# uniio/ivf-hnsw

Measured on AMD Instinct MI355X. Metric: queries/sec @ Recall@1, SIFT1B PQ16 nprobe=32; ADC scan HBM GB/s vs peak, higher is better.
Workload: dtype f32

## Files before the change

### ivf-hnsw_amd/csrc/capi_internal.h

```cpp
#pragma once
#include "../../include/ivfhnsw_hip.h"
#include "ivfhnsw_kernels.h"

#include <hip/hip_runtime.h>

#include <algorithm>
#include <new>
#include <cmath>
#include <cstddef>
#include <cstdio>
#include <cstdlib>
#include <cstring>
#include <functional>
#include <string>
#include <unordered_map>
#include <vector>

namespace ivfhnsw_gpu_impl {

int fail(int code, const char *fmt, ...) __attribute__((format(printf, 2, 3)));

#define HIP_TRY(expr)                                                                                        \
    do {                                                                                                     \
        hipError_t e_ = (expr);                                                                              \
// ... 98 lines not shown
};

struct StatusWords {
    uint32_t bits;
    uint32_t walk_next;
    uint32_t redo_len;
    uint32_t redo_next;
    uint32_t redo_exits;
    uint32_t heap_redo_len;
    uint32_t heap_redo_exits;
    uint32_t pad;
};
static_assert(offsetof(StatusWords, redo_len) == offsetof(StatusWords, walk_next) + 4 &&
                  offsetof(StatusWords, redo_next) == offsetof(StatusWords, walk_next) + 8 &&
                  offsetof(StatusWords, redo_exits) == offsetof(StatusWords, walk_next) + 12,
              "launch_coarse: next_query is followed by the three words of the redo header");
static_assert(offsetof(StatusWords, heap_redo_exits) == offsetof(StatusWords, heap_redo_len) + 4, "launch_heap_scan: redo_hdr[0..1]");
static_assert(offsetof(StatusWords, bits) == 0 && sizeof(StatusWords) == 8 * sizeof(uint32_t), "8 words, bits first");

struct WalkScratch {
    bool zero = false;
    void *zero_ptr = nullptr;
    size_t zero_bytes = 0;
    bool counters_clean = true;
};

}

using namespace ivfhnsw_gpu_impl;

#define IVFHNSW_GPU_DEVBUFS(X) \
    X(goff) X(loff) X(cnorm) X(pqc) X(ntab) X(opq_at) X(opq_a) X(codes) X(ncodes) X(ids)  \
    X(g_alpha) X(g_nn) X(g_sizes) X(g_inter)  \
    X(q_counts) X(q_links) X(q_vectors) X(q_qrows) X(q_nbrows) X(q_nbnorms) X(q_fat) X(q_links_c)  \
    X(e_pqc) X(e_ntab) X(e_a) X(e_at) X(e_x) X(e_idx) X(e_dist) X(e_res) X(e_tmp) X(e_codes) X(e_ncodes)  \
    X(t_x) X(t_y) X(t_cb) X(t_assign) X(t_part) X(t_c)  \
    X(k_q) X(k_x) X(k_qn) X(k_xn) X(k_part) X(k_ids) X(k_dists)  \
    X(km_x) X(km_c) X(km_assign) X(km_dist) X(km_cnt) X(km_start) X(km_ids) X(km_ids2) X(km_hist) X(km_part) X(km_status) X(km_pairs)  \
    X(gb_table) X(gb_fwd) X(gb_fcnt) X(gb_deg) X(gb_roff) X(gb_ids) X(gb_ids2) X(gb_hist) X(gb_stat) X(gb_counts) X(gb_links)  \
    X(cg_q) X(cg_cidx) X(cg_ids) X(cg_dists) X(gc_nn) X(cg_cvn) X(cg_tab) X(cg_tab2) X(cg_off) X(cg_alpha2) X(cg_sub)  \
    X(base_rows) X(base_stage)  \
    X(r_q) X(r_cand) X(r_dist) X(r_lab)  \
    X(ex_q) X(ex_part) X(ex_raw) X(ex_dist) X(ex_lab)  \
    X(ap_idx) X(ap_ids) X(ap_codes) X(ap_ncodes) X(ap_cnt) X(ap_own) X(ap_part) X(ap_status) X(ap_perm) X(ap_perm2) X(ap_hist) X(ap_tiles)  \
    X(gp_sub) X(gp_sizes) X(gp_pre_old) X(gp_pre_new) X(gp_rows) X(gp_gather) X(ga_cidx) X(ga_off) X(ga_nn) X(ga_alpha) X(ga_inter) X(ga_status)  \
    X(rm_labels) X(rm_bits) X(rm_mask) X(rm_keep) X(rm_rem) X(rm_out) X(rm_part) X(rm_status) X(rm_sizes)  \
    X(f_mask) X(f_count)  \
    X(fs_planes) X(fs_count) X(fs_qslots)  \
    X(tg_table) X(tg_rows)  \
    X(bf_words) X(bf_rows) X(bf_own) X(bf_count)  \
    X(bs_table) X(bs_plan) X(bs_qslots)  \
    X(bt_tags) X(bt_rows) X(bt_off) X(bt_work)  \
    X(w_xq) X(w_luts) X(w_segs) X(w_lpos) X(w_hdr) X(w_keys) X(w_cid) X(w_cd) X(w_qsd) X(w_totals) X(w_visited) X(w_status) X(w_stream) X(w_slen) X(w_tail) X(w_redo) X(w_hredo) X(w_heap)  \
    X(rg_dist) X(rg_lab) X(rg_slices) X(rg_part) X(rg_lims)  \
    X(xr_dist) X(xr_lab) X(xr_slices) X(xr_part) X(xr_map) X(xr_lims) X(xr_tot)  \
    X(lc_bits) X(lc_labels) X(lc_sorted) X(lc_perm) X(lc_perm2) X(lc_hist) X(lc_lo) X(lc_cnt) X(lc_rows) X(lc_counts) X(lc_scalar)  \
    X(rc_rows) X(rc_y) X(rc_out) X(sr_keys) X(sr_rows)  \
    X(s_q) X(s_cid) X(s_cd) X(s_dist) X(s_lab) X(s_keys) X(s_len)

struct ivfhnsw_gpu {
    int device = 0;
    hipStream_t stream = nullptr;
    bool own_stream = false;
    bool is_view = false;

#define IVFHNSW_X(name) DevBuf name;
    IVFHNSW_GPU_DEVBUFS(IVFHNSW_X)
// ... 320 lines not shown
```

### ivf-hnsw_amd/csrc/capi_upload.cpp

```cpp
#include "capi_internal.h"
#include "walk_form.h"

namespace {

int check_desc(const ivfhnsw_ivf_desc *d, bool need_lists)
{
    if (!d)
        return fail(IVFHNSW_ERR_INVALID, "null descriptor");
    if (d->d == 0 || d->nc == 0 || d->code_size == 0)
        return fail(IVFHNSW_ERR_INVALID, "d, nc and code_size must be positive");
    if (d->code_size % 4)
        return fail(IVFHNSW_ERR_INVALID, "code_size %zu is not a multiple of 4 (IndexIVF_HNSW.cpp:805)", d->code_size);
    if (d->code_size * 1024 > kScanDynLdsMax)
        return fail(IVFHNSW_ERR_INVALID, "code_size %zu: the query's table (1 KB per code byte) must fit %zu KB of LDS",
                    d->code_size, kScanDynLdsMax / 1024);
    if (d->d % d->code_size)
        return fail(IVFHNSW_ERR_INVALID, "d %zu is not a multiple of code_size %zu", d->d, d->code_size);
    if (d->d / d->code_size > 64)
        return fail(IVFHNSW_ERR_INVALID, "sub-vector dimension %zu > 64 unsupported", d->d / d->code_size);
    if (d->nc >= 0xffffffffull)
        return fail(IVFHNSW_ERR_INVALID, "nc too large");
    if (!d->offsets || !d->centroid_norms || !d->pq_centroids || !d->norm_table)
        return fail(IVFHNSW_ERR_INVALID, "offsets, centroid_norms, pq_centroids and norm_table are required");
    if (need_lists && d->offsets[d->nc] != 0 && (!d->ids || !d->codes || !d->norm_codes))
        return fail(IVFHNSW_ERR_INVALID, "ids, codes and norm_codes are required");
    if (d->shard_world == 0 || d->shard_rank >= d->shard_world)
        return fail(IVFHNSW_ERR_INVALID, "bad shard %u of %u", d->shard_rank, d->shard_world);
    if (d->offsets[0] != 0)
        return fail(IVFHNSW_ERR_INVALID, "offsets[0] must be 0");
    for (size_t c = 0; c < d->nc; c++)
        if (d->offsets[c + 1] < d->offsets[c])
            return fail(IVFHNSW_ERR_INVALID, "offsets not monotone at list %zu", c);
    return IVFHNSW_OK;
// ... 251 lines not shown
    h->g.nsubc = (int)nsubc;
    h->g.alphas = h->g_alpha.as<float>();
    h->g.nn_idx = h->g_nn.as<uint32_t>();
    h->g.sub_sizes = h->g_sizes.as<uint32_t>();
    h->g.inter_dists = h->g_inter.as<float>();
    h->g.dedupe = grouping_dedupe(nc, nsubc, subgroup_sizes, nn_centroid_idxs);
    h->has_group = true;
    return IVFHNSW_OK;
} catch (const std::bad_alloc &) {
    return fail(IVFHNSW_ERR_NOMEM, "ivfhnsw_gpu_upload_grouping: host allocation failed");
}

static int build_byte_rows(ivfhnsw_gpu *h, size_t n, size_t d, const float *vectors)
{
    static const bool off = [] {
        const char *e = getenv("IVFHNSW_WALK_PREFILTER");
        return e && atoi(e) == 0;
    }();
    if (off || d > 2048)
        return IVFHNSW_OK;
    float lo = vectors[0], hi = vectors[0];
    bool finite = true;
    for (size_t i = 0; i < n * d; i++) {
        const float v = vectors[i];
        finite &= std::isfinite(v);
        lo = std::min(lo, v);
        hi = std::max(hi, v);
    }
    const float step = (float)(((double)hi - (double)lo) / 255.0);
    if (!finite || !(step > 0.f) || !std::isfinite(step) || !std::isfinite(1.f / step))
        return IVFHNSW_OK;
    std::vector<uint8_t> rows(n * d);
    double worst = 0.0;
    for (size_t r = 0; r < n; r++) {
        double e2 = 0.0;
        for (size_t j = 0; j < d; j++) {
            const double x = vectors[r * d + j];
            double c = std::nearbyint((x - (double)lo) / (double)step);
            c = std::min(255.0, std::max(0.0, c));
            rows[r * d + j] = (uint8_t)c;
            const double e = x - ((double)lo + (double)step * c);
            e2 += e * e;
        }
        worst = std::max(worst, e2);
    }
    const double errc = std::sqrt(worst) / (double)step * (1.0 + 1e-6) + 1e-6;
    float errc_f = (float)errc;
    if ((double)errc_f < errc)
        errc_f = std::nextafter(errc_f, INFINITY);
    int rc = upload(h->q_qrows, rows.data(), n * d);
    if (rc)
        return rc;
    h->gr.qrows = h->q_qrows.as<uint8_t>();
    h->gr.q_lo = lo;
    h->gr.q_step = step;
    h->gr.q_errc = errc_f;
    return IVFHNSW_OK;
}

static int build_neighbour_rows(ivfhnsw_gpu *h)
{
    static const int mode = [] {
        const char *e = getenv("IVFHNSW_WALK_PREFILTER");
        return e ? atoi(e) : 2;
    }();
    static const double cap_gib = [] {
        const char *e = getenv("IVFHNSW_WALK_NBROWS_GIB");
        return e ? atof(e) : 48.0;
    }();
    if (!h->gr.qrows || mode != 2 || h->gr.d > 128 || h->gr.n >= (1u << 24) || h->gr.maxM > 64)
        return IVFHNSW_OK;
    const int nb_rows = (h->gr.maxM + 31) & ~31;
    const size_t bytes = (size_t)h->gr.n * nb_rows * 128;
    if ((double)bytes > cap_gib * 1073741824.0)
        return IVFHNSW_OK;
    int rc = h->q_nbrows.ensure(bytes);
    if (rc)
        return rc;
    if ((rc = h->q_nbnorms.ensure((size_t)h->gr.n * nb_rows * sizeof(uint32_t))))
        return rc;
    if ((rc = h->q_links_c.ensure((size_t)h->gr.n * h->gr.maxM * sizeof(uint32_t))))
        return rc;
    HIP_TRY(launch_build_nbrows(h->stream, h->gr, h->q_nbrows.as<uint8_t>(), h->q_nbnorms.as<uint32_t>(), nb_rows,
                                h->q_links_c.as<uint32_t>()));
    HIP_TRY(hipStreamSynchronize(h->stream));
    h->gr.nbrows = h->q_nbrows.as<uint8_t>();
    h->gr.nbnorms = h->q_nbnorms.as<uint32_t>();
    h->gr.links_c = h->q_links_c.as<uint32_t>();
    h->gr.nb_rows = nb_rows;
    return IVFHNSW_OK;
}

int ivfhnsw_gpu_upload_quantizer(ivfhnsw_gpu *h, size_t n, size_t d, size_t maxM, uint32_t enterpoint,
                                 const uint8_t *link_counts, const uint32_t *links, const float *vectors)
try {
    int rc = table_change_guard(h, kUploads, "upload_quantizer", false);
    if (rc)
        return rc;
    if (n == 0 || d == 0 || maxM == 0 || maxM > 255 || n >= 0xffffffffull || enterpoint >= n || !link_counts ||
        !links || !vectors)
        return fail(IVFHNSW_ERR_INVALID, "bad quantizer arrays (n %zu, d %zu, maxM %zu)", n, d, maxM);
    if (d % 16)
        return fail(IVFHNSW_ERR_INVALID, "d %zu: the reference distance ignores dims beyond a multiple of 16 "
                                         "(hnswalg.cpp:330); only multiples of 16 are supported here", d);
    bool unique = true;
    uint32_t tmp[256];
    for (size_t i = 0; i < n; i++) {
        if (link_counts[i] > maxM)
            return fail(IVFHNSW_ERR_INVALID, "node %zu has %u links > maxM %zu", i, link_counts[i], maxM);
        for (size_t j = 0; j < link_counts[i]; j++)
            if (links[i * maxM + j] >= n)
                return fail(IVFHNSW_ERR_INVALID, "node %zu link %zu out of range", i, j);
        if (unique && link_counts[i] > 1) {
            const size_t c = link_counts[i];
            std::copy(links + i * maxM, links + i * maxM + c, tmp);
            std::sort(tmp, tmp + c);
            unique = std::adjacent_find(tmp, tmp + c) == tmp + c;
// ... 29 lines not shown
    if ((rc = upload(h->q_vectors, vectors, n * d * sizeof(float))))
        return rc;
    h->gr.n = (uint32_t)n;
    h->gr.d = (int)d;
    h->gr.maxM = (int)maxM;
    h->gr.enterpoint = enterpoint;
    h->gr.counts = h->q_counts.as<uint8_t>();
    h->gr.links = h->q_links.as<uint32_t>();
    h->gr.vectors = h->q_vectors.as<float>();
    {
        static const int merge = [] {
            const char *e = getenv("IVFHNSW_WALK_MERGE");
            return (e && atoi(e) == 0) ? 0 : 1;
        }();
        h->gr.merge_admissions = merge;
    }
    {
        static const int late_knob = [] {
            const char *e = getenv("IVFHNSW_WALK_LATE_VISIT");
            return e ? (atoi(e) != 0 ? 1 : 0) : -1;
        }();
        const bool late = late_knob < 0 ? walk_late_visit_default(n) : late_knob == 1;
        h->gr.links_unique = (unique && late) ? 1 : 0;
    }
    h->gr.fat = nullptr;
    h->gr.qrows = nullptr;
    h->gr.nbrows = nullptr;
    h->gr.nbnorms = nullptr;
    h->gr.links_c = nullptr;
    h->gr.nb_rows = 0;
    h->gr.q_lo = 0.f;
    h->gr.q_step = 1.f;
    h->gr.q_errc = 0.f;
    if ((rc = build_byte_rows(h, n, d, vectors)))
        return rc;
    if ((rc = build_neighbour_rows(h)))
        return rc;
    h->has_graph = true;
    return IVFHNSW_OK;
} catch (const std::bad_alloc &) {
    return fail(IVFHNSW_ERR_NOMEM, "ivfhnsw_gpu_upload_quantizer: host allocation failed");
}

int ivfhnsw_gpu_prepare_latency(ivfhnsw_gpu *h)
{
    if (h && h->is_view)
        return fail(IVFHNSW_ERR_STATE, "prepare_latency goes to the handle that holds the tables, not to a view of it");
    int rc = bind(h);
    if (rc)
        return rc;
    if (!h->has_graph)
        return fail(IVFHNSW_ERR_STATE, "prepare_latency needs upload_quantizer");
    if (h->gr.fat)
        return IVFHNSW_OK;
    GraphTables probe = h->gr;
    probe.fat = reinterpret_cast<const float *>(h);
    if (!coarse_latency_supported(probe, 1))
        return fail(IVFHNSW_ERR_INVALID, "the latency walk needs d = 128 or 96, maxM <= 32 and at most 2^20 nodes "
                                         "(have d %d, maxM %d, %u nodes); small batches keep the throughput walk",
                    h->gr.d, h->gr.maxM, h->gr.n);
    if ((rc = h->q_fat.ensure(coarse_latency_fat_bytes(h->gr))))
        return rc;
    HIP_TRY(launch_build_fat(h->stream, h->gr, h->q_fat.as<float>()));
    HIP_TRY(hipStreamSynchronize(h->stream));
    h->gr.fat = h->q_fat.as<float>();
    return IVFHNSW_OK;
// ... 68 lines not shown
```

### ivf-hnsw_amd/csrc/ivfhnsw_kernels.h

```cpp
#pragma once

#include <hip/hip_runtime.h>
#include <mutex>
#include <stdint.h>

#include "scan_dispatch.h"
#include "sweep_plan_math.h"
#include "update_math.h"
#include "walk_form.h"

namespace ivfhnsw_gpu_impl {

struct DynLdsState {
    std::mutex m;
    size_t raised[64] = {};
};
inline hipError_t raise_dyn_lds(const void *kern, size_t bytes, DynLdsState &st)
{
    int dev = 0;
    hipError_t e = hipGetDevice(&dev);
    if (e != hipSuccess)
        return e;
    if (dev < 0 || dev >= 64)
        return hipFuncSetAttribute(kern, hipFuncAttributeMaxDynamicSharedMemorySize, (int)bytes);
// ... 60 lines not shown
struct IvfTables {
    int d, M, dsub;
    uint32_t nc;
    const uint64_t *goff;
    const uint32_t *loff;
    const float *centroid_norms;
    const float *pq_centroids;
    const float *norm_table;
    const float *opq_At;
    const uint8_t *codes;
    const uint8_t *norm_codes;
    const uint32_t *ids;
    uint32_t shard_rank, shard_world;
};

struct GroupTables {
    int nsubc;
    const float *alphas;
    const uint32_t *nn_idx;
    const uint32_t *sub_sizes;
    const float *inter_dists;
    int dedupe;
};

struct GraphTables {
    uint32_t n;
    int d, maxM;
    uint32_t enterpoint;
    const uint8_t *counts;
    const uint32_t *links;
    const float *vectors;
    const uint8_t *qrows;
    float q_lo, q_step, q_errc;
    const uint8_t *nbrows;
    const uint32_t *nbnorms;
    const uint32_t *links_c;
    int nb_rows;
    const float *fat;
    int visited_clean;
    int merge_admissions;
    int links_unique;
};

hipError_t launch_opq(hipStream_t s, const float *At, const float *x, float *y, int nq, int d);
hipError_t launch_lut(hipStream_t s, const IvfTables &t, const float *xq, float *luts, int nq, const PlanHdr *hdr = nullptr);
hipError_t launch_plan_ivf(hipStream_t s, const IvfTables &t, const uint32_t *coarse_ids, const float *coarse_dists,
                           int nprobe, uint64_t max_codes, const PlanView &p, uint64_t *keys, int k);
hipError_t launch_plan_lut(hipStream_t s, const IvfTables &t, const float *xq, const uint32_t *coarse_ids,
                           const float *coarse_dists, int nprobe, uint64_t max_codes, const PlanView &p, uint64_t *keys,
                           int k, float *luts);
hipError_t launch_plan_grouping(hipStream_t s, const IvfTables &t, const GroupTables &g, const GraphTables &gr,
                                const float *xq, const uint32_t *coarse_ids, const float *coarse_dists, int nprobe,
                                uint64_t max_codes, int do_pruning, const PlanView &p, uint64_t *keys, int k,
                                float *qsd_scratch);
struct ScanOut {
    uint64_t *stream = nullptr;
    uint32_t *stream_len = nullptr;
    uint32_t stream_cap = 0;
    float *sel_dist = nullptr;
    int64_t *sel_labels = nullptr;
};
hipError_t launch_scan(hipStream_t s, const IvfTables &t, const float *luts, const PlanView &p, int k, int nsplit,
                       uint64_t *keys, int seg_len_hint, const ScanFilter &fmask, const ScanOut &out, bool *did_select,
                       const char **kernel_name);
bool scan_pipe_supported(const IvfTables &t, int max_seg, int nq, int nsplit, bool has_codes, bool forced = false);
hipError_t launch_scan_pipe(hipStream_t s, const IvfTables &t, const float *xq, const PlanView &p, uint64_t *keys);
// ... 55 lines not shown
                               uint32_t *cnt, double *part, uint32_t *status);
hipError_t launch_scan_u32(hipStream_t s, const uint32_t *in, uint32_t *out, size_t len);
hipError_t launch_sort_by_key(hipStream_t s, const uint32_t *keys, size_t n, int key_bits, uint32_t *ids_a, uint32_t *ids_b,
                              uint32_t *hist, uint32_t **sorted);
hipError_t launch_sort_by_key_from(hipStream_t s, const uint32_t *keys, size_t n, int key_bits, const uint32_t *start,
                                   uint32_t *ids_a, uint32_t *ids_b, uint32_t *hist, uint32_t **sorted);
hipError_t launch_kmeans_means(hipStream_t s, const float *x, size_t n, const uint32_t *members, const uint32_t *start,
                               const uint32_t *cnt, float *c, size_t nc, int d);
hipError_t launch_kmeans_split(hipStream_t s, float *c, const uint32_t *pairs, size_t npairs, int d);
inline int knn_splits_for(size_t nq, size_t nx) { return sweep_splits_for(nq, nx, 128); }
hipError_t launch_knn_norms(hipStream_t s, const float *x, float *out, size_t n, int d);
hipError_t launch_knn(hipStream_t s, const float *Q, const float *X, const float *qn, const float *xn, size_t nq, size_t nx,
                      int d, int k, int mode, int nsplit, unsigned long long *part, uint32_t *ids, float *dists);
size_t graph_forward_lds_bytes(int d, int ncand);
size_t graph_fold_lds_bytes(int d, int maxM);
hipError_t launch_graph_forward(hipStream_t s, const float *x, const uint32_t *table, size_t n, int d, int M, int ncand,
                                uint32_t *fwd, uint8_t *fcnt, uint32_t *deg);
hipError_t launch_graph_fold(hipStream_t s, const float *x, const uint32_t *fwd, const uint8_t *fcnt, const uint32_t *roff,
                             const uint32_t *pairs, size_t n, int d, int M, int maxM, uint8_t *counts, uint32_t *links,
                             uint32_t *longest);
hipError_t launch_group_table(hipStream_t s, int mode, const float *vectors, const uint32_t *centroid_idx,
                              const uint32_t *nn, const float *alphas, const float *cv_in, float *out, size_t ngroups,
                              int nsubc, int d);
size_t group_points_lds_bytes(int nsubc, int d);
hipError_t launch_group_points(hipStream_t s, int mode, const float *vectors, const uint32_t *centroid_idx,
                               const float *table, const float *cv_norms, const unsigned long long *offsets,
                               const float *x, float *out_num, float *out_den, uint32_t *out_sub, size_t ngroups,
                               int nsubc, int d);
hipError_t launch_group_alpha(hipStream_t s, const unsigned long long *offsets, const float *num, const float *den,
                              float *alphas, size_t ngroups);
hipError_t launch_group_rows(hipStream_t s, const unsigned long long *offsets, const uint32_t *sub, uint32_t *rows,
                             size_t ngroups, int nsubc);
hipError_t launch_build_nbrows(hipStream_t s, const GraphTables &g, uint8_t *nbrows, uint32_t *nbnorms, int nb_rows,
                               uint32_t *links_c);
hipError_t launch_fill_bytes(hipStream_t s, uint8_t *dst, size_t nbytes, uint64_t seed);
hipError_t launch_fill_iota(hipStream_t s, uint32_t *dst, size_t n, uint32_t first);
hipError_t launch_fill_lists(hipStream_t s, const IvfTables &t, uint8_t *codes, uint8_t *norm_codes, uint32_t *ids,
                             uint64_t seed_codes, uint64_t seed_norms);
hipError_t launch_rerank_permute(hipStream_t s, const uint8_t *src, size_t src_stride, uint8_t *dst, size_t count, int d);
size_t rerank_lds_bytes(int kc, int d);
hipError_t launch_rerank(hipStream_t s, const uint8_t *base, uint64_t n, int d, const float *queries,
                         const int64_t *cand, size_t nq, int kc, int k, float *dist, int64_t *labels);
inline int exact_rows_per_block(int k) { return k <= 32 ? 128 : 64; }
inline int exact_splits_for(size_t nq, size_t nx, int k) { return sweep_splits_for(nq, nx, exact_rows_per_block(k)); }
hipError_t launch_exact_search(hipStream_t s, const uint8_t *Qp, const uint8_t *X, size_t nq, size_t nx, int d, int k,
                               int nsplit, unsigned long long *part, float *dists, int64_t *labels, const SweepCols &cols = {});
constexpr int kExactRangeMaxShift = 20;
inline int exact_range_map_words(size_t nx, int nsplit, int map_shift) { return sweep_map_words(nx, nsplit, map_shift); }
hipError_t launch_exact_range(hipStream_t s, bool fill, const uint8_t *Qp, const uint8_t *X, size_t nq, size_t q_off, size_t nx,
                              int d, int thr, int nsplit, uint32_t *slices, unsigned long long *total, uint32_t *map,
                              int map_shift, float *dist, int64_t *labels, size_t out_cap, const SweepCols &cols = {});
hipError_t launch_pass_words(hipStream_t s, const uint32_t *bits, size_t bit_words, uint64_t n, int deny, uint32_t *words,
                             unsigned long long *count);
hipError_t launch_pass_rows(hipStream_t s, const uint32_t *words, uint64_t n, uint32_t *cnt, uint32_t *part, uint32_t *rows);
hipError_t launch_strip_plan(hipStream_t s, const uint8_t *d_slots, size_t m, const StripCols *table, void *plan, size_t bound,
                             StripPlan *sp);
hipError_t launch_rerank_permute_rows(hipStream_t s, const uint8_t *src, size_t src_stride, uint8_t *dst, size_t count, int d,
                                      const int32_t *row_src);
hipError_t launch_exact_search_strips(hipStream_t s, const uint8_t *Qp, const uint8_t *X, size_t nq, size_t bound, int d, int k,
                                      int nsplit, unsigned long long *part, float *dists, int64_t *labels, const StripPlan &sp,
                                      unsigned forms);
hipError_t launch_exact_range_strips(hipStream_t s, bool fill, const uint8_t *Qp, const uint8_t *X, size_t bound, size_t q_off,
                                     size_t nx, int d, int thr, int nsplit, uint32_t *slices, unsigned long long *total,
                                     uint32_t *map, int map_shift, float *dist, int64_t *labels, size_t out_cap,
                                     const StripPlan &sp, unsigned forms);
hipError_t launch_base_tags_apply(hipStream_t s, const uint32_t *rows, const uint16_t *vals, size_t cnt, uint64_t n, uint16_t *tags,
                                  uint32_t *conflict);
// ... 74 lines not shown
```

### ivf-hnsw_amd/csrc/kernels_hnsw.hip

```cpp
#include "ivfhnsw_kernels.h"
#include "device_common.h"
#include "walk_set.h"
#include "walk_form.h"

#include <float.h>
#include <stdio.h>
#include <stdlib.h>
#include <type_traits>

namespace ivfhnsw_gpu_impl {


template <int TAGW> struct VisFields {
    static constexpr int cntw = TAGW == 8 ? 8 : TAGW == 10 ? 14 : 16;
    static constexpr int cshift = 64 - cntw;
    static constexpr int slots = cshift / TAGW;
    static constexpr unsigned long long ones()
    {
        unsigned long long o = 0;
        for (int i = 0; i < slots; i++)
            o |= 1ull << (TAGW * i);
        return o;
    }
};

template <int TAGW, int NB>
__device__ __forceinline__ bool visit_test_and_set(uint32_t id, unsigned long long *vt, uint32_t *bm, bool &used_bitmap)
{
    if constexpr (TAGW != 0) {
        using F = VisFields<TAGW>;
        constexpr unsigned long long kOnes = F::ones();
        constexpr unsigned long long kHighs = kOnes << (TAGW - 1);
        const uint32_t b = id % (uint32_t)NB;
        const unsigned long long tag = (unsigned long long)((id / (uint32_t)NB) + 1);
        const unsigned long long old = vt[b];
        const unsigned long long x = old ^ (tag * kOnes);
// ... 66 lines not shown
        __builtin_amdgcn_sched_barrier(0);
#pragma unroll
        for (int i = 0; i < 4; i++) {
            if (j0 + 2 * i < nchunk) {
                const float4 *qq = reinterpret_cast<const float4 *>(sqp + 16 * (j0 + 2 * i));
                const uint32_t ws[4] = {w[i].x, w[i].y, w[i].z, w[i].w};
#pragma unroll
                for (int c = 0; c < 4; c++) {
                    const float4 qv = qq[c];
                    const float t0 = qv.x - (float)(ws[c] & 0xffu);
                    const float t1 = qv.y - (float)((ws[c] >> 8) & 0xffu);
                    const float t2 = qv.z - (float)((ws[c] >> 16) & 0xffu);
                    const float t3 = qv.w - (float)(ws[c] >> 24);
                    a0 = fmaf(t0, t0, a0);
                    a1 = fmaf(t1, t1, a1);
                    a2 = fmaf(t2, t2, a2);
                    a3 = fmaf(t3, t3, a3);
                }
            }
        }
    }
    return (a0 + a1) + (a2 + a3);
}

__device__ __forceinline__ unsigned long long walk_stamp()
{
    __builtin_amdgcn_sched_barrier(0);
    const unsigned long long t = __builtin_amdgcn_s_memtime();
    __builtin_amdgcn_s_waitcnt(0xC07F);
    __builtin_amdgcn_sched_barrier(0);
    return t;
}


struct WalkArgs {
    GraphTables g;
    const float *xq;
    int nq, nprobe, ef;
    uint32_t *coarse_ids;
    float *coarse_dists;
    uint32_t *visited;
    size_t vwords;
    uint32_t *status, *next_query, *redo_hdr, *redo_list;
    uint32_t *tail_bitmaps;
    unsigned long long *stamp_out;
};

template <class T> __device__ __forceinline__ const __attribute__((address_space(4))) T *late_kernarg()
{
    auto p = (const __attribute__((address_space(4))) T *)__builtin_amdgcn_kernarg_segment_ptr();
    asm volatile("" : "+s"(p));
    return p;
}

template <int NCH, int TAGW, int FMODE, bool STAMPS = false, bool SPILL = false, int D = 0, int MAXM = 0, bool MERGE = true>
__global__ __launch_bounds__(64, 4) void hnsw_walk_kernel(WalkArgs a)
{
    constexpr bool SHAPED = D != 0 && MAXM != 0;
    const GraphTables &g = a.g;
    const int ef = a.ef;
    uint32_t *__restrict__ const visited = a.visited;
    const size_t vwords = a.vwords;
#define WALK_COLD(f) (SHAPED ? late_kernarg<WalkArgs>()->f : a.f)
    extern __shared__ __attribute__((aligned(16))) unsigned char smem[];
    float *s_q = reinterpret_cast<float *>(smem);
    static_assert(!SHAPED || (FMODE >= 2 && !SPILL && D % 16 == 0 && D <= 128 && MAXM <= 64),
                  "shape constants go with the neighbour-row forms");
    static_assert(SHAPED || MERGE, "the generic form reads merge_admissions at run time");
    const int dim = D ? D : g.d;
    const int maxm = MAXM ? MAXM : g.maxM;
    const int nbr_rows = MAXM ? (MAXM + 31) / 32 * 32 : g.nb_rows;
    float *s_qp = s_q + dim;
    const int dp = FMODE == 1 ? dim : 0;
    uint32_t *s_q8 = reinterpret_cast<uint32_t *>(s_qp + dp);
    unsigned long long *tail = reinterpret_cast<unsigned long long *>(smem + (size_t)(dim + dp) * sizeof(float) + 512);
    constexpr int NB = walk_vis_buckets(TAGW);
    unsigned long long st_acc[9] = {0, 0, 0, 0, 0, 0}, st_t = 0;
    const int merge_extra = (NCH <= 4 && ef + 8 > kTailCap) ? ef + 8 - kTailCap : 0;
    unsigned long long *vt = tail + kTailCap + merge_extra;
    constexpr bool LDSVIS = TAGW != 0;

    const int lane = threadIdx.x;
    const int judged_row = 8 * (((lane >> 2) & 1) * 2 + (lane & 1)) + (lane >> 3);
    const bool merge_on = SHAPED ? MERGE : g.merge_admissions != 0;
    constexpr bool prefilter = FMODE != 0;
    constexpr bool inline_rows = FMODE >= 2;
    constexpr bool ROWNORMS = FMODE == 3;
    constexpr bool CK = FMODE >= 2;
    auto enc_id = [](uint32_t id, uint32_t c) { return CK ? (id << 7) | c : id; };
    auto dec_id = [](uint32_t e) { return CK ? e >> 7 : e; };
    uint32_t *bm = visited + (size_t)blockIdx.x * vwords;
    TailSpill spill;
    spill.bm = SPILL ? a.tail_bitmaps + (size_t)blockIdx.x * vwords : nullptr;
    spill.hi = -1;
    spill.count = 0;
    bool bitmap_dirty = !(LDSVIS && g.visited_clean);
    bool redo_ran = false;

    for (;;) {
        int q = 0;
        if constexpr (SPILL) {
            if (lane == 0) {
                const uint32_t i = atomicAdd(&a.redo_hdr[1], 1u);
                q = i < a.redo_hdr[0] ? (int)a.redo_list[i] : a.nq;
            }
        } else {
            if (lane == 0)
                q = (int)atomicAdd(WALK_COLD(next_query), 1u);
        }
        q = __builtin_amdgcn_readfirstlane(q);
        if (q >= WALK_COLD(nq))
            break;
        redo_ran = true;
        if (STAMPS)
            st_t = walk_stamp();

        if (!LDSVIS || bitmap_dirty) {
            uint4 *bm4 = reinterpret_cast<uint4 *>(bm);
            const size_t v4 = vwords / 4;
            for (size_t w = lane; w < v4; w += 64)
                bm4[w] = make_uint4(0u, 0u, 0u, 0u);
            bitmap_dirty = false;
        }
        if (LDSVIS)
            for (int w = lane; w < NB; w += 64)
                vt[w] = 0ull;
        __syncthreads();
        float qp_sq = 0.f;
        for (int i = lane; i < dim; i += 64) {
            const float v = WALK_COLD(xq)[(size_t)q * dim + i];
            s_q[i] = v;
            if (prefilter) {
                const float vp = __fdiv_rn(__fsub_rn(v, WALK_COLD(g.q_lo)), g.q_step);
                if (!inline_rows)
                    s_qp[i] = vp;
                qp_sq = fmaf(vp, vp, qp_sq);
            }
        }
        __syncthreads();
        float q_reg[16];
#pragma unroll
        for (int i = 0; i < 16; i++)
            if constexpr (D != 0)
                q_reg[i] = 8 * i < D ? s_q[8 * i + (lane & 7)] : 0.f;
            else
                q_reg[i] = (g.d == 128 || g.d == 96) && 8 * i < g.d ? s_q[8 * i + (lane & 7)] : 0.f;
        float pf_slack = 0.f, pf_slack_q = 0.f, pf_bonus = 0.f;
        int q16_w = 0;
        int x_const = 0;
        bool x_any = false;
        bool x_hi = false;
        uint4 qp_h = make_uint4(0u, 0u, 0u, 0u), qp_l = qp_h, qp_x = qp_h;
        if (prefilter) {
#pragma unroll
            for (int off = 32; off > 0; off >>= 1)
                qp_sq += __shfl_xor(qp_sq, off, 64);
            pf_slack = __uint_as_float(__builtin_amdgcn_readfirstlane(__float_as_uint(WALK_COLD(g.q_errc) + 3.9e-6f * sqrtf(qp_sq))));
            if (inline_rows) {
                float dq_sq = 0.f, bonus = 0.f;
                int s_hh = 0, s_hl = 0, s_ll = 0, s_xh = 0, s_xl = 0;
                if (lane < 32) {
                    uint32_t wh = 0, wl = 0, wxl = 0, wxh = 0;
#pragma unroll
                    for (int b = 0; b < 4; b++) {
                        const int comp = 4 * lane + b;
                        const float vp = comp < dim ? __fdiv_rn(__fsub_rn(s_q[comp], WALK_COLD(g.q_lo)), g.q_step) : 0.f;
                        const float fh = fminf(255.f, fmaxf(0.f, floorf(vp)));
                        const float fl = fminf(255.f, fmaxf(0.f, rintf((vp - fh) * 256.f)));
                        const float qin = fh + fl * 0.00390625f;
                        const bool below = vp < 0.f, above = vp >= 256.f;
                        const float e = (below || above) ? 0.f : vp - qin;
                        dq_sq = fmaf(e, e, dq_sq);
                        const float out = (below || above) ? fabsf(vp - qin) : 0.f;
                        bonus = fmaf(out, out, bonus);
                        const int x = (int)fminf(255.f, floorf(2.f * out));
                        const int hi = (int)fh, lo = (int)fl;
                        s_hh += hi * hi;
                        s_hl += hi * lo;
                        s_ll += lo * lo;
                        wh |= (uint32_t)hi << (8 * b);
                        wl |= (uint32_t)lo << (8 * b);
                        if (below)
                            wxl |= (uint32_t)x << (8 * b);
                        if (above)
                            wxh |= (uint32_t)x << (8 * b);
                        s_xl += below ? x : 0;
                        s_xh += above ? x : 0;
                    }
                    s_q8[lane] = wh;
                    s_q8[32 + lane] = wl;
// ... 202 lines not shown
                        const uint32_t ws[4] = {nw[i].x, nw[i].y, nw[i].z, nw[i].w};
                        uint32_t hr = 0, rr = 0;
#pragma unroll
                        for (int c = 0; c < 4; c++) {
                            hr = __builtin_amdgcn_udot4(qh[c], ws[c], hr, false);
                            if constexpr (!ROWNORMS)
                                rr = __builtin_amdgcn_udot4(ws[c], ws[c], rr, false);
                        }
                        uint32_t lr = hr << 8;
#pragma unroll
                        for (int c = 0; c < 4; c++)
                            lr = __builtin_amdgcn_udot4(ql[c], ws[c], lr, false);
                        S[i] = (int)(128u * rr - lr);
                        X[i] = 0;
                        if (x_any) {
                            uint32_t xlr = 0, xhr = 0;
#pragma unroll
                            for (int c = 0; c < 4; c++)
                                xlr = __builtin_amdgcn_udot4(xl[c], ws[c], xlr, false);
                            if (x_hi) {
                                asm volatile("" ::);
#pragma unroll
                                for (int c = 0; c < 4; c++)
                                    xhr = __builtin_amdgcn_udot4(xh[c], ws[c], xhr, false);
                            }
                            X[i] = (int)(xlr - xhr);
                        }
                    }
                    int mine, minex = 0;
                    if (x_any)
                        oct_sum4x2(S, X, lane, mine, minex);
                    else
                        mine = oct_sum4(S, lane);
                    mine += (int)(128u * row_rr);
                    const float m1 = fmaxf(
                        0.f, __builtin_amdgcn_sqrtf((float)(mine + q16_w) * 0.0078125f) * 0.9990234375f - pf_slack_q);
                    const float m2 = fmaf(m1, m1, fmaf((float)(minex + x_const), 0.9990234375f, pf_bonus));
                    const float m = fmaxf(0.f, __builtin_amdgcn_sqrtf(m2) * 0.9990234375f - pf_slack) * g.q_step;
                    const float lb = m * m * 0.9990234375f;
                    const unsigned long long dropm = __ballot(lb > worst) & 0x3333333333333333ull;
                    const int rel = lane - rb;
                    const int ri = rel >> 3;
                    if (rel >= 0 && rel < 32 && ((dropm >> (8 * (rel & 7) + 4 * (ri >> 1) + (ri & 1))) & 1ull))
                        fresh = false;
                    rb += 32;
                    if (rb >= cnt)
                        break;
                    if constexpr (CK) {
                        const uint4 *nbr =
                            reinterpret_cast<const uint4 *>(g.nbrows + (size_t)node * nbr_rows * 128) + (lane & 7);
                        const int last = max(cnt - 1, 0);
#pragma unroll
                        for (int i = 0; i < 4; i++)
                            if (rb + 8 * i < cnt)
                                nw[i] = nbr[min(rb + 8 * i + (lane >> 3), last) * 8];
                    } else {
                        const uint4 *nbr =
                            reinterpret_cast<const uint4 *>(g.nbrows + ((size_t)node * nbr_rows + rb) * 128) + lane;
#pragma unroll
                        for (int i = 0; i < 4; i++)
                            nw[i] = nbr[i * 64];
                    }
                    if constexpr (ROWNORMS)
                        row_rr = g.nbnorms[(size_t)node * nbr_rows + rb + judged_row];
                }
                mask = __ballot(fresh);
                nfresh = __popcll(mask);
                if (filter_first) {
                    pend = fresh;
                    pend_full = full_now;
                    pend_id = nb;
                    pend_any = nfresh > 0;
                }
            } else if (filter_now && nfresh > 0) {
                const float worst = __uint_as_float(key_dist_bits(last_now));
                const int myrow = __popcll(mask & ((1ull << lane) - 1ull));
                for (int base = 0; base < nfresh; base += 32) {
                    const int r = base + (lane >> 1);
                    const bool active = r < nfresh;
                    const int src = active ? nth_set_bit(mask, r) : 0;
                    const uint32_t nbq = (uint32_t)__shfl((int)nb, src, 64);
                    float S = 0.f;
                    if (active)
                        S = byte_row_dist_half(g.qrows + (size_t)nbq * dim, s_qp, dim, lane & 1);
                    S += __shfl_xor(S, 1, 64);
                    const float m = fmaxf(0.f, __builtin_amdgcn_sqrtf(S) * 0.9990234375f - pf_slack) * g.q_step;
                    const float lb = m * m * 0.9990234375f;
                    const unsigned long long drop = __ballot(active && lb > worst);
                    const int rel = myrow - base;
                    if (fresh && rel >= 0 && rel < 32 && ((drop >> (2 * rel)) & 1ull))
                        fresh = false;
                }
                mask = __ballot(fresh);
                nfresh = __popcll(mask);
            }
            if (STAMPS) {
                const unsigned long long t = walk_stamp();
                st_acc[1] += t - st_t;
                st_t = t;
            }

            unsigned long long rest = mask;
            for (int base = 0; base < nfresh && ntail >= 0; base += 8) {
                const int r = base + (lane >> 3);
                const bool active = r < nfresh;
                const int src = take8_set_bits(rest, lane);
                const uint32_t nbe = (uint32_t)__shfl((int)nb_enc, src, 64);
                const uint32_t nbq = dec_id(nbe);
                float dq = 0.f;
                if (active) {
                    if constexpr (D != 0)
                        dq = l2_ref_order_oct_regs<D / 8>(g.vectors + (size_t)nbq * D, q_reg, lane & 7);
                    else
                        dq = g.d == 128  ? l2_ref_order_oct_regs<16>(g.vectors + (size_t)nbq * 128, q_reg, lane & 7)
                             : g.d == 96 ? l2_ref_order_oct_regs<12>(g.vectors + (size_t)nbq * 96, q_reg, lane & 7)
                                         : l2_ref_order_oct(g.vectors + (size_t)nbq * g.d, s_q, g.d, lane & 7);
                }
                if (STAMPS) {
                    asm volatile("s_waitcnt vmcnt(0)" ::: "memory");
                    const unsigned long long t = walk_stamp();
// ... 137 lines not shown
                }
            }
        }
    }
    if constexpr (SPILL) {
        if (lane == 0) {
            __threadfence();
            if (atomicAdd(&a.redo_hdr[2], 1u) == gridDim.x - 1) {
                a.redo_hdr[-1] = 0;
                a.redo_hdr[0] = 0;
                a.redo_hdr[1] = 0;
                a.redo_hdr[2] = 0;
            }
        }
    }
    if (SPILL && redo_ran) {
        uint4 *bm4 = reinterpret_cast<uint4 *>(bm);
        for (size_t w = lane; w < vwords / 4; w += 64)
            bm4[w] = make_uint4(0u, 0u, 0u, 0u);
    }
    if (LDSVIS && bitmap_dirty) {
        uint4 *bm4 = reinterpret_cast<uint4 *>(bm);
        for (size_t w = lane; w < vwords / 4; w += 64)
            bm4[w] = make_uint4(0u, 0u, 0u, 0u);
    }
    if (STAMPS && a.stamp_out && lane == 0)
        for (int i = 0; i < 9; i++)
            atomicAdd(&a.stamp_out[i], st_acc[i]);
#undef WALK_COLD
}

__global__ __launch_bounds__(64) void build_nbrows_kernel(GraphTables g, uint8_t *__restrict__ nbrows,
                                                          uint32_t *__restrict__ nbnorms, int nb_rows,
                                                          uint32_t *__restrict__ links_c)
{
    const size_t node = blockIdx.x;
    const int cnt = g.counts[node];
    if ((int)threadIdx.x < g.maxM) {
        uint32_t e = 0;
        if ((int)threadIdx.x < cnt) {
            const uint32_t id = g.links[node * g.maxM + threadIdx.x];
            e = id | ((uint32_t)g.counts[id] << 24);
        }
        links_c[node * g.maxM + threadIdx.x] = e;
    }
    const int cpr = g.d >> 4;
    for (int r0 = 0; r0 < nb_rows; r0 += 8) {
        const int r = r0 + (threadIdx.x >> 3), c = threadIdx.x & 7;
        uint4 v = make_uint4(0u, 0u, 0u, 0u);
        if (r < cnt && c < cpr)
            v = reinterpret_cast<const uint4 *>(g.qrows + (size_t)g.links[node * g.maxM + r] * g.d)[c];
        reinterpret_cast<uint4 *>(nbrows + (node * nb_rows + r) * 128)[c] = v;
        uint32_t rr = 0;
        rr = __builtin_amdgcn_udot4(v.x, v.x, rr, false);
        rr = __builtin_amdgcn_udot4(v.y, v.y, rr, false);
        rr = __builtin_amdgcn_udot4(v.z, v.z, rr, false);
        rr = __builtin_amdgcn_udot4(v.w, v.w, rr, false);
        rr = (uint32_t)oct_sum((int)rr);
        if (c == 0)
            nbnorms[node * nb_rows + r] = rr;
    }
}

hipError_t launch_build_nbrows(hipStream_t s, const GraphTables &g, uint8_t *nbrows, uint32_t *nbnorms, int nb_rows,
                               uint32_t *links_c)
{
    if (!g.qrows || g.d > 128 || (g.d & 15) || nb_rows < g.maxM || (nb_rows & 31) || g.n >= (1u << 24) || g.maxM > 64)
        return hipErrorInvalidValue;
    hipLaunchKernelGGL(build_nbrows_kernel, dim3(g.n), dim3(64), 0, s, g, nbrows, nbnorms, nb_rows, links_c);
    return hipGetLastError();
}

static const WalkKnobs &walk_knobs()
{
    static const WalkKnobs knobs = [] {
        auto num = [](const char *knob, int unset) { return getenv(knob) ? atoi(getenv(knob)) : unset; };
        const char *vis = getenv("IVFHNSW_WALK_VIS");
        const int w = num("IVFHNSW_WALK_TAGW", 0);
        return WalkKnobs{vis && vis[0] == 'b', (w == 10 || w == 12 || w == 16) ? w : 0, num("IVFHNSW_WALK_SHAPE", 1) != 0,
                         num("IVFHNSW_WALK_STAMPS", 0) == 1};
    }();
    return knobs;
}

static WalkGraph walk_graph_of(const GraphTables &g)
{
    return {g.n, g.d, g.maxM, g.nb_rows, g.qrows != nullptr, g.nbrows != nullptr, g.links_unique != 0, g.merge_admissions != 0};
}

hipError_t launch_coarse(hipStream_t s, const GraphTables &g_in, const float *xq, int nq, int nprobe, int ef,
                         uint32_t *coarse_ids, float *coarse_dists, uint32_t *visited_scratch,
                         size_t visited_words_per_slot, int nslots, uint32_t *status, uint32_t *next_query,
                         size_t visited_bytes, bool *visited_zero, uint32_t *redo_list, uint32_t *tail_bitmaps,
                         int tail_slots, bool *counters_clean)
{
    if (nq == 0)
        return hipSuccess;
    GraphTables g = g_in;
    if (ef > 1024 || ef < 1 || nprobe > ef || g.maxM > 64 || g.n >= 0x80000000u || (visited_words_per_slot & 3) ||
        !redo_list || !tail_bitmaps || tail_slots < 1)
        return hipErrorInvalidValue;
    uint32_t *redo_hdr = next_query + 1;
// ... 80 lines not shown
```

Before: 6.551 million.

## Tighten HNSW walk prefilter bound with per-row quantization error codes

After: 6.631 million, median of 6. 1.2% higher.

```diff
diff --git a/ivf-hnsw_amd/csrc/capi_internal.h b/ivf-hnsw_amd/csrc/capi_internal.h
--- a/ivf-hnsw_amd/csrc/capi_internal.h
+++ b/ivf-hnsw_amd/csrc/capi_internal.h
@@ -154,7 +154,7 @@
 #define IVFHNSW_GPU_DEVBUFS(X) \
     X(goff) X(loff) X(cnorm) X(pqc) X(ntab) X(opq_at) X(opq_a) X(codes) X(ncodes) X(ids)  \
     X(g_alpha) X(g_nn) X(g_sizes) X(g_inter)  \
-    X(q_counts) X(q_links) X(q_vectors) X(q_qrows) X(q_nbrows) X(q_nbnorms) X(q_fat) X(q_links_c)  \
+    X(q_counts) X(q_links) X(q_vectors) X(q_qrows) X(q_nbrows) X(q_nbnorms) X(q_fat) X(q_links_c) X(q_rowerr)  \
     X(e_pqc) X(e_ntab) X(e_a) X(e_at) X(e_x) X(e_idx) X(e_dist) X(e_res) X(e_tmp) X(e_codes) X(e_ncodes)  \
     X(t_x) X(t_y) X(t_cb) X(t_assign) X(t_part) X(t_c)  \
     X(k_q) X(k_x) X(k_qn) X(k_xn) X(k_part) X(k_ids) X(k_dists)  \
diff --git a/ivf-hnsw_amd/csrc/capi_upload.cpp b/ivf-hnsw_amd/csrc/capi_upload.cpp
--- a/ivf-hnsw_amd/csrc/capi_upload.cpp
+++ b/ivf-hnsw_amd/csrc/capi_upload.cpp
@@ -1,4 +1,5 @@
 #include "capi_internal.h"
+#include "walk_bound.h"
 #include "walk_form.h"
 
 namespace {
@@ -316,6 +317,7 @@
         return IVFHNSW_OK;
     std::vector<uint8_t> rows(n * d);
     double worst = 0.0;
+    std::vector<double> row_e2(n);
     for (size_t r = 0; r < n; r++) {
         double e2 = 0.0;
         for (size_t j = 0; j < d; j++) {
@@ -326,19 +328,27 @@
             const double e = x - ((double)lo + (double)step * c);
             e2 += e * e;
         }
+        row_e2[r] = e2;
         worst = std::max(worst, e2);
     }
-    const double errc = std::sqrt(worst) / (double)step * (1.0 + 1e-6) + 1e-6;
+    const double errc = walk_err_round_up(worst, (double)step);
     float errc_f = (float)errc;
     if ((double)errc_f < errc)
         errc_f = std::nextafter(errc_f, INFINITY);
+    const float unit = walk_err_unit(errc_f);
+    std::vector<uint16_t> codes(n);
+    for (size_t r = 0; r < n; r++)
+        codes[r] = (uint16_t)walk_err_code(walk_err_round_up(row_e2[r], (double)step), unit);
     int rc = upload(h->q_qrows, rows.data(), n * d);
     if (rc)
+        return rc;
+    if ((rc = upload(h->q_rowerr, codes.data(), n * sizeof(uint16_t))))
         return rc;
     h->gr.qrows = h->q_qrows.as<uint8_t>();
     h->gr.q_lo = lo;
     h->gr.q_step = step;
     h->gr.q_errc = errc_f;
+    h->gr.q_errunit = unit;
     return IVFHNSW_OK;
 }
 
@@ -366,7 +376,7 @@
     if ((rc = h->q_links_c.ensure((size_t)h->gr.n * h->gr.maxM * sizeof(uint32_t))))
         return rc;
     HIP_TRY(launch_build_nbrows(h->stream, h->gr, h->q_nbrows.as<uint8_t>(), h->q_nbnorms.as<uint32_t>(), nb_rows,
-                                h->q_links_c.as<uint32_t>()));
+                                h->q_links_c.as<uint32_t>(), h->q_rowerr.as<uint16_t>()));
     HIP_TRY(hipStreamSynchronize(h->stream));
     h->gr.nbrows = h->q_nbrows.as<uint8_t>();
     h->gr.nbnorms = h->q_nbnorms.as<uint32_t>();
@@ -462,6 +472,7 @@
     h->gr.q_lo = 0.f;
     h->gr.q_step = 1.f;
     h->gr.q_errc = 0.f;
+    h->gr.q_errunit = 0.f;
     if ((rc = build_byte_rows(h, n, d, vectors)))
         return rc;
     if ((rc = build_neighbour_rows(h)))
diff --git a/ivf-hnsw_amd/csrc/ivfhnsw_kernels.h b/ivf-hnsw_amd/csrc/ivfhnsw_kernels.h
--- a/ivf-hnsw_amd/csrc/ivfhnsw_kernels.h
+++ b/ivf-hnsw_amd/csrc/ivfhnsw_kernels.h
@@ -116,6 +116,7 @@
     const float *vectors;
     const uint8_t *qrows;
     float q_lo, q_step, q_errc;
+    float q_errunit;
     const uint8_t *nbrows;
     const uint32_t *nbnorms;
     const uint32_t *links_c;
@@ -237,7 +238,7 @@
 hipError_t launch_group_rows(hipStream_t s, const unsigned long long *offsets, const uint32_t *sub, uint32_t *rows,
                              size_t ngroups, int nsubc);
 hipError_t launch_build_nbrows(hipStream_t s, const GraphTables &g, uint8_t *nbrows, uint32_t *nbnorms, int nb_rows,
-                               uint32_t *links_c);
+                               uint32_t *links_c, const uint16_t *row_err);
 hipError_t launch_fill_bytes(hipStream_t s, uint8_t *dst, size_t nbytes, uint64_t seed);
 hipError_t launch_fill_iota(hipStream_t s, uint32_t *dst, size_t n, uint32_t first);
 hipError_t launch_fill_lists(hipStream_t s, const IvfTables &t, uint8_t *codes, uint8_t *norm_codes, uint32_t *ids,
diff --git a/ivf-hnsw_amd/csrc/kernels_hnsw.hip b/ivf-hnsw_amd/csrc/kernels_hnsw.hip
--- a/ivf-hnsw_amd/csrc/kernels_hnsw.hip
+++ b/ivf-hnsw_amd/csrc/kernels_hnsw.hip
@@ -2,6 +2,7 @@
 #include "device_common.h"
 #include "walk_set.h"
 #include "walk_form.h"
+#include "walk_bound.h"
 
 #include <float.h>
 #include <stdio.h>
@@ -134,6 +135,10 @@
     return t;
 }
 
+
+struct HwSqrt {
+    __device__ __forceinline__ float operator()(float v) const { return __builtin_amdgcn_sqrtf(v); }
+};
 
 struct WalkArgs {
     GraphTables g;
@@ -188,6 +193,7 @@
     constexpr bool prefilter = FMODE != 0;
     constexpr bool inline_rows = FMODE >= 2;
     constexpr bool ROWNORMS = FMODE == 3;
+    constexpr bool TIGHT = FMODE >= 2 && D != 0;
     constexpr bool CK = FMODE >= 2;
     auto enc_id = [](uint32_t id, uint32_t c) { return CK ? (id << 7) | c : id; };
     auto dec_id = [](uint32_t e) { return CK ? e >> 7 : e; };
@@ -247,7 +253,7 @@
                 q_reg[i] = 8 * i < D ? s_q[8 * i + (lane & 7)] : 0.f;
             else
                 q_reg[i] = (g.d == 128 || g.d == 96) && 8 * i < g.d ? s_q[8 * i + (lane & 7)] : 0.f;
-        float pf_slack = 0.f, pf_slack_q = 0.f, pf_bonus = 0.f;
+        float pf_slack = 0.f, pf_unit = 0.f, pf_slack_q = 0.f, pf_bonus = 0.f;
         int q16_w = 0;
         int x_const = 0;
         bool x_any = false;
@@ -257,7 +263,10 @@
 #pragma unroll
             for (int off = 32; off > 0; off >>= 1)
                 qp_sq += __shfl_xor(qp_sq, off, 64);
-            pf_slack = __uint_as_float(__builtin_amdgcn_readfirstlane(__float_as_uint(WALK_COLD(g.q_errc) + 3.9e-6f * sqrtf(qp_sq))));
+            pf_slack = __uint_as_float(__builtin_amdgcn_readfirstlane(
+                __float_as_uint((ROWNORMS ? 0.f : WALK_COLD(g.q_errc)) + 3.9e-6f * sqrtf(qp_sq))));
+            if constexpr (ROWNORMS)
+                pf_unit = WALK_COLD(g.q_errunit);
             if (inline_rows) {
                 float dq_sq = 0.f, bonus = 0.f;
                 int s_hh = 0, s_hl = 0, s_ll = 0, s_xh = 0, s_xl = 0;
@@ -526,12 +535,10 @@
                         oct_sum4x2(S, X, lane, mine, minex);
                     else
                         mine = oct_sum4(S, lane);
-                    mine += (int)(128u * row_rr);
-                    const float m1 = fmaxf(
-                        0.f, __builtin_amdgcn_sqrtf((float)(mine + q16_w) * 0.0078125f) * 0.9990234375f - pf_slack_q);
-                    const float m2 = fmaf(m1, m1, fmaf((float)(minex + x_const), 0.9990234375f, pf_bonus));
-                    const float m = fmaxf(0.f, __builtin_amdgcn_sqrtf(m2) * 0.9990234375f - pf_slack) * g.q_step;
-                    const float lb = m * m * 0.9990234375f;
+                    mine += (int)(128u * walk_norm_of(row_rr));
+                    const float slack = ROWNORMS ? walk_row_slack(row_rr, pf_unit, pf_slack) : pf_slack;
+                    const float lb = walk_lb_int<TIGHT>(mine + q16_w, minex + x_const, pf_slack_q, pf_bonus, slack, g.q_step,
+                                                        HwSqrt());
                     const unsigned long long dropm = __ballot(lb > worst) & 0x3333333333333333ull;
                     const int rel = lane - rb;
                     const int ri = rel >> 3;
@@ -578,8 +585,7 @@
                     if (active)
                         S = byte_row_dist_half(g.qrows + (size_t)nbq * dim, s_qp, dim, lane & 1);
                     S += __shfl_xor(S, 1, 64);
-                    const float m = fmaxf(0.f, __builtin_amdgcn_sqrtf(S) * 0.9990234375f - pf_slack) * g.q_step;
-                    const float lb = m * m * 0.9990234375f;
+                    const float lb = walk_lb_of_root<false>(__builtin_amdgcn_sqrtf(S), pf_slack, g.q_step);
                     const unsigned long long drop = __ballot(active && lb > worst);
                     const int rel = myrow - base;
                     if (fresh && rel >= 0 && rel < 32 && ((drop >> (2 * rel)) & 1ull))
@@ -783,7 +789,8 @@
 
 __global__ __launch_bounds__(64) void build_nbrows_kernel(GraphTables g, uint8_t *__restrict__ nbrows,
                                                           uint32_t *__restrict__ nbnorms, int nb_rows,
-                                                          uint32_t *__restrict__ links_c)
+                                                          uint32_t *__restrict__ links_c,
+                                                          const uint16_t *__restrict__ row_err)
 {
     const size_t node = blockIdx.x;
     const int cnt = g.counts[node];
@@ -809,16 +816,16 @@
         rr = __builtin_amdgcn_udot4(v.w, v.w, rr, false);
         rr = (uint32_t)oct_sum((int)rr);
         if (c == 0)
-            nbnorms[node * nb_rows + r] = rr;
+            nbnorms[node * nb_rows + r] = walk_norm_pack(rr, r < cnt ? (uint32_t)row_err[g.links[node * g.maxM + r]] : 0u);
     }
 }
 
 hipError_t launch_build_nbrows(hipStream_t s, const GraphTables &g, uint8_t *nbrows, uint32_t *nbnorms, int nb_rows,
-                               uint32_t *links_c)
-{
-    if (!g.qrows || g.d > 128 || (g.d & 15) || nb_rows < g.maxM || (nb_rows & 31) || g.n >= (1u << 24) || g.maxM > 64)
+                               uint32_t *links_c, const uint16_t *row_err)
+{
+    if (!g.qrows || !row_err || g.d > 128 || (g.d & 15) || nb_rows < g.maxM || (nb_rows & 31) || g.n >= (1u << 24) || g.maxM > 64)
         return hipErrorInvalidValue;
-    hipLaunchKernelGGL(build_nbrows_kernel, dim3(g.n), dim3(64), 0, s, g, nbrows, nbnorms, nb_rows, links_c);
+    hipLaunchKernelGGL(build_nbrows_kernel, dim3(g.n), dim3(64), 0, s, g, nbrows, nbnorms, nb_rows, links_c, row_err);
     return hipGetLastError();
 }
 
diff --git a/ivf-hnsw_amd/csrc/walk_bound.h b/ivf-hnsw_amd/csrc/walk_bound.h
--- /dev/null
+++ b/ivf-hnsw_amd/csrc/walk_bound.h
@@ -0,0 +1,71 @@
+#pragma once
+#include <math.h>
+#include <stdint.h>
+
+#if defined(__HIPCC__) || defined(__CUDACC__)
+#define WALK_BOUND_HD __host__ __device__ __forceinline__
+#else
+#define WALK_BOUND_HD inline
+#endif
+
+namespace ivfhnsw_gpu_impl {
+
+constexpr float kWalkMarginWide = 0.9990234375f;
+
+template <bool TIGHT>
+struct WalkMargins {
+    static constexpr float k1 = TIGHT ? 0.99999809265136719f : kWalkMarginWide;
+    static constexpr float k2 = TIGHT ? 0.99999904632568359f : kWalkMarginWide;
+    static constexpr float k3 = TIGHT ? 0.99999618530273438f : kWalkMarginWide;
+    static constexpr float k4 = TIGHT ? 0.99998474121093750f : kWalkMarginWide;
+};
+
+constexpr uint32_t kWalkNormBits = 23, kWalkNormMask = (1u << kWalkNormBits) - 1u, kWalkErrCodes = 511;
+
+WALK_BOUND_HD uint32_t walk_norm_pack(uint32_t norm, uint32_t code) { return norm | (code << kWalkNormBits); }
+WALK_BOUND_HD uint32_t walk_norm_of(uint32_t entry) { return entry & kWalkNormMask; }
+WALK_BOUND_HD float walk_row_slack(uint32_t entry, float unit, float slack_query)
+{
+    return fmaf((float)(entry >> kWalkNormBits), unit, slack_query);
+}
+
+inline float walk_err_unit(float errc)
+{
+    const double u = (double)errc / (double)kWalkErrCodes;
+    float f = (float)u;
+    while ((double)f * (double)kWalkErrCodes < (double)errc)
+        f = nextafterf(f, INFINITY);
+    return f;
+}
+
+inline uint32_t walk_err_code(double err_row, float unit)
+{
+    if (!(err_row > 0.0))
+        return 0;
+    double e = ceil(err_row / (double)unit);
+    if (!(e < (double)kWalkErrCodes))
+        return kWalkErrCodes;
+    uint32_t code = (uint32_t)e;
+    while (code < kWalkErrCodes && (double)code * (double)unit < err_row)
+        code++;
+    return code;
+}
+
+inline double walk_err_round_up(double err2, double step) { return sqrt(err2) / step * (1.0 + 1e-6) + 1e-6; }
+
+template <bool TIGHT>
+WALK_BOUND_HD float walk_lb_of_root(float root, float slack, float step)
+{
+    const float m = fmaxf(0.f, root * WalkMargins<TIGHT>::k3 - slack) * step;
+    return m * m * WalkMargins<TIGHT>::k4;
+}
+
+template <bool TIGHT, class Sqrt>
+WALK_BOUND_HD float walk_lb_int(int w, int x, float slack_q, float bonus, float slack, float step, Sqrt root)
+{
+    const float m1 = fmaxf(0.f, root((float)w * 0.0078125f) * WalkMargins<TIGHT>::k1 - slack_q);
+    const float m2 = fmaf(m1, m1, fmaf((float)x, WalkMargins<TIGHT>::k2, bonus));
+    return walk_lb_of_root<TIGHT>(root(m2), slack, step);
+}
+
+}
```
